# mattreturn1/ComputerVision_ObjectDetection_FeatureMatching

Measured on AMD Instinct MI355X. Metric: matches+homographies/sec (10k x 10k SIFT, 50k RANSAC iters) at 1/2/4/8 GPUs, higher is better.
Workload: dtype i8-MFMA exact-int distances (i32 acc), fp64 DLT/Jacobi, fp32 reprojection; 1 GPU; c4: one global batch of 256 scenes x 1 model set, 10000x10000 descriptors, maxIters 50000, scenes sharded over 1 GPU(s) (256 on rank 0); problems_per_gpu=256, global_batch=256, parallelism=dp1, batches_in_flight=16, dist_backend=nccl, hw_queues=24

## Files before the change

computervision_objectdetection_featurematching_amd/csrc/api.cpp:

```cpp
#include <hip/hip_runtime.h>

#include <algorithm>
#include <cfloat>
#include <climits>
#include <cmath>
#include <cstdarg>
#include <cstdio>
#include <cstdlib>
#include <cstring>
#include <map>
#include <mutex>
#include <string>
#include <vector>

#include "../../include/mim.h"
#include "../../include/mim_detect.hpp"
#include "knn_coll.h"
#include "mim_internal.h"
#include "radius.h"

namespace mim {
void launch_prep_batch(const PrepJob* jobs, int njobs, int total_tiles, hipStream_t st);
void launch_knn(const ProbDev* probs, const KnnWork* works, int n_works, const int* seg_start, int n_blocks, Top2* parts,
                int* dyn_ctr, float kappa, float flip_ratio, hipStream_t st);
// ... 152 lines not shown
        if (err != hipSuccess || ab + bb == 0) return;
        if (ab) memcpy(p + off, a, ab);
        if (bb) memcpy(p + off + ab, b, bb);
        err = hipMemcpyAsync(dst, p + off, ab + bb, hipMemcpyHostToDevice, s);
        off += ab + bb;
    }
    template <class T> void put(const DevBuf& dst, const std::vector<T>& v) { put(dst.p, v.data(), vec_bytes(v)); }
    hipError_t done() { return err != hipSuccess ? err : ps.release_after(s); }
};

}

namespace mim {
struct RansacWs {
    DevBuf state, samples, hyp, counts, bounds, flags, irr_bits, irr, irr_cnt, cls, cls_tab, pass_bits, defer, defer_n, chains, best_h, cand, ncand, cex, cH, decided, stream,
        scratch, inl, tiles, tbox, perm, surv, nsurv, err;
    long long stream_len = 0;
};
}

struct mim_ctx {
    int device = 0;
    hipStream_t own = nullptr, stream = nullptr;
    std::mutex mu;
    std::string err;
    Arena arena;
    std::vector<SetRec> sets;
    DevBuf probs, works, parts, good_q, good_t, pts, n_good, results, masks, knn_idx, knn_dist, inl_tab, inl_out, knn_ctr, ham_works, flt_works;
    RansacWs rws;
    std::vector<ProbDev> h_probs;
    int n_ham_works = 0;
// ... 141 lines not shown
    (void)hipStreamSynchronize(c->stream);
    for (auto& e : c->evs) (void)hipEventDestroy(e.e);
    for (hipEvent_t e : c->ev_pool) (void)hipEventDestroy(e);
    if (c->samp) (void)hipStreamSynchronize(c->samp);
    if (c->ev_samp_fork) (void)hipEventDestroy(c->ev_samp_fork);
    for (auto e : c->ev_samp)
        if (e) (void)hipEventDestroy(e);
    if (c->samp) (void)hipStreamDestroy(c->samp);
    mim::sift_ws_destroy(c->sift);
    for (mim::SiftWs* w : c->sift_scales) mim::sift_ws_destroy(w);
    c->stage.destroy();
    c->prep_stage.destroy();
    c->arena.release();
    for (DevBuf* b : {&c->probs, &c->works, &c->parts, &c->good_q, &c->good_t, &c->pts, &c->n_good,
                      &c->results, &c->masks, &c->knn_idx, &c->knn_dist, &c->inl_tab, &c->inl_out, &c->knn_ctr, &c->ham_works, &c->flt_works, &c->ham_cross_works, &c->colmin, &c->cross_tab, &c->topk_parts, &c->topk_ham_works, &c->topk_flt_works, &c->topk_probs, &c->coll_parts, &c->coll_ham_works, &c->coll_flt_works, &c->coll_i8_probs, &c->coll_i8_works, &c->coll_tab, &c->coll_queries, &c->rad_counts, &c->rad_cursor, &c->rad_offsets, &c->rad_meta, &c->rad_keys, &c->rad_scratch, &c->rad_ham_works, &c->rad_flt_works, &c->rad_i8_works, &c->rad_probs, &c->rws.state, &c->rws.samples,
                      &c->rws.hyp, &c->rws.counts, &c->rws.bounds, &c->rws.flags, &c->rws.irr_bits, &c->rws.irr, &c->rws.irr_cnt, &c->rws.cls, &c->rws.cls_tab, &c->rws.pass_bits, &c->rws.defer, &c->rws.defer_n, &c->rws.chains, &c->rws.best_h, &c->rws.cand, &c->rws.ncand, &c->rws.cex, &c->rws.cH, &c->rws.decided, &c->rws.stream, &c->rws.scratch, &c->rws.inl, &c->rws.tiles, &c->rws.tbox, &c->rws.perm, &c->rws.surv, &c->rws.nsurv, &c->rws.err, &c->prep_jobs})
        b->release();
    if (c->own) (void)hipStreamDestroy(c->own);
    delete c;
}

const char* mim_last_error(const mim_ctx* c) { return c ? c->err.c_str() : "null ctx"; }

mim_status mim_ctx_set_stream(mim_ctx* c, void* stream) {
    if (!c) return MIM_EINVAL;
    std::lock_guard<std::mutex> lk(c->mu);
    c->stream = stream ? (hipStream_t)stream : c->own;
    return MIM_OK;
}

mim_status mim_ctx_set_sampler_stream(mim_ctx* c, int32_t on) {
// ... 1523 lines not shown
    HIPCHK(c, c->rws.defer_n.ensure(sizeof(int) * (size_t)std::max(n, 1) * def_rounds));
    HIPCHK(c, c->rws.chains.ensure(ransac_chain_bytes() * (size_t)std::max(n, 1)));
    HIPCHK(c, c->rws.best_h.ensure(sizeof(double) * 9 * std::max(n, 1)));
    const size_t cap = (size_t)std::max(n, 1) * 2 * kCandPerProblem;
    HIPCHK(c, c->rws.cand.ensure(sizeof(int) * cap));
    HIPCHK(c, c->rws.ncand.ensure(sizeof(int) * 2 * std::max(n, 1)));
    HIPCHK(c, c->rws.cex.ensure(sizeof(int) * cap));
    HIPCHK(c, c->rws.cH.ensure(sizeof(double) * 9 * cap));
    HIPCHK(c, c->rws.decided.ensure(sizeof(int) * cap));
    HIPCHK(c, c->rws.inl.ensure(sizeof(float4) * good_total));
    HIPCHK(c, c->rws.tiles.ensure(sizeof(uint4) * 128 * ((good_total + 31) / 32)));
    HIPCHK(c, c->rws.tbox.ensure(sizeof(float4) * ((good_total + 31) / 32)));
    HIPCHK(c, c->rws.perm.ensure(sizeof(int) * 2 * good_total));
    HIPCHK(c, c->rws.surv.ensure(sizeof(int) * it_total));
    HIPCHK(c, c->rws.nsurv.ensure(sizeof(int) * std::max(n, 1)));
    HIPCHK(c, c->rws.err.ensure(sizeof(int) * 4));
    HIPCHK(c, c->results.ensure(sizeof(mim_result) * std::max(n, 1)));
    HIPCHK(c, c->masks.ensure(good_total));
    HIPCHK(c, hipMemsetAsync(c->rws.err.p, 0, sizeof(int) * 4, c->stream));
    b = RansacBufs{};
    b.state = c->rws.state.as<RansacState>();
    b.samples = c->rws.samples.as<int4>();
    b.hyp = c->rws.hyp.as<float>();
    b.counts = c->rws.counts.as<int>();
    b.bounds = c->rws.bounds.as<int2>();
    b.flags = c->rws.flags.as<uint8_t>();
    b.irr_bits = c->rws.irr_bits.as<uint8_t>();
    b.best_h = c->rws.best_h.as<double>();
    b.cand = c->rws.cand.as<int>();
    b.ncand = c->rws.ncand.as<int>();
// ... 9 lines not shown
    const char* cde = getenv("MIM_CHECK_DEFER");
    b.def_rounds = (cde && cde[0] == '0') ? 0 : def_rounds;
    b.irr_blocks = irr_blocks;
    b.cls = c->rws.cls.as<SamplerClass>();
    b.cls_tab = c->rws.cls_tab.as<SamplerClassSlot>();
    b.cls_tab_n = q_max + 1;
    b.chains = c->rws.chains.p;
    b.stream = c->rws.stream.as<uint32_t>();
    b.stream_len = c->rws.stream_len;
    b.inl = c->rws.inl.as<float4>();
    b.tiles = c->rws.tiles.as<uint4>();
    b.tbox = c->rws.tbox.as<float4>();
    b.perm = c->rws.perm.as<int>();
    b.surv = c->rws.surv.as<int>();
    b.nsurv = c->rws.nsurv.as<int>();
    b.err = c->rws.err.as<int>();
    if (c->samp_on < 0) {
        const char* e = getenv("MIM_SAMPLER_STREAM");
        c->samp_on = (e && e[0] == '0') ? 0 : 1;
    }
    if (c->samp_on && !c->samp) {
        HIPCHK(c, hipStreamCreateWithFlags(&c->samp, hipStreamNonBlocking));
        HIPCHK(c, hipEventCreateWithFlags(&c->ev_samp_fork, hipEventDisableTiming));
        for (auto& e : c->ev_samp) HIPCHK(c, hipEventCreateWithFlags(&e, hipEventDisableTiming));
    }
    b.s2 = c->samp_on ? c->samp : nullptr;
    b.ev_fork = c->ev_samp_fork;
    b.ev_samp[0] = c->ev_samp[0];
    b.ev_samp[1] = c->ev_samp[1];
    rp = RansacParams{};
// ... 19 lines not shown
    g.flag_cap = (long long)np * flag_per;
    g.irr += (long long)p0 * b.irr_blocks * kIrrCap;
    g.irr_cnt += (long long)p0 * b.irr_blocks;
    g.cls += p0;
    g.pass_bits += (long long)p0 * flag_per / 32;
    g.defer += (long long)p0 * b.def_rounds * kRansacDefSlots;
    g.defer_n += (long long)p0 * b.def_rounds;
    g.chains = static_cast<char*>(b.chains) + (size_t)p0 * ransac_chain_bytes();
    g.best_h += 9LL * p0;
    g.cand += (long long)p0 * 2 * kCandPerProblem;
    g.ncand += 2 * p0;
    g.cex += (long long)p0 * 2 * kCandPerProblem;
    g.cH += 9LL * p0 * 2 * kCandPerProblem;
    g.decided += (long long)p0 * 2 * kCandPerProblem;
    g.nsurv += p0;
    ransac_enqueue(rp, np, c->probs.as<ProbDev>() + p0, c->pts.as<float4>(), c->n_good.as<int>() + p0, g,
                   c->masks.as<uint8_t>(), c->results.as<mim_result>() + p0, raw, c->cur, mark_cb, c, c->exact_all);
    HIPCHK(c, hipGetLastError());
    return MIM_OK;
}

static mim_status ransac_locked(mim_ctx* c, int n, const mim_params* prm, int raw) {
    RansacBufs b;
    RansacParams rp;
    long long flag_per = 0;
    mim_status s = ransac_prepare(c, n, prm, b, rp, flag_per);
    if (s != MIM_OK) return s;
    c->cur = c->stream;
    return ransac_enqueue_range(c, 0, n, b, rp, flag_per, raw);
}
// ... 243 lines not shown
```

computervision_objectdetection_featurematching_amd/csrc/mim_internal.h:

```cpp
#pragma once
#include <hip/hip_runtime.h>
#include <stdint.h>

#include "knn_schedule.h"
#include "knn_topk_merge.h"

namespace mim {

constexpr int kDim = 128;
constexpr int kTileRows = 64;
constexpr int kTileBytes = kTileRows * kDim;
constexpr int kNormWords = 4 * kTileRows;
constexpr int kWave = 64;
#ifndef MIM_KNN_STAGE
#define MIM_KNN_STAGE 4
#endif
constexpr int kKnnStage = MIM_KNN_STAGE;

struct SetDev {
    const int8_t* frag;
    const int* norm;
    const float* f32;
    const float2* kp;
    int n;
// ... 179 lines not shown
    int2* defer;
    int* defer_n;
    int def_rounds;
    int irr_blocks;
    SamplerClass* cls;
    SamplerClassSlot* cls_tab;
    int cls_tab_n;
    const uint32_t* stream;
    long long stream_len;
    float4* inl;
    uint4* tiles;
    float4* tbox;
    int* perm;
    int* surv;
    int* nsurv;
    int* err;
    hipStream_t s2;
    hipEvent_t ev_fork;
    hipEvent_t ev_samp[2];
};
}

#include <string>
#include <vector>
#include "../../include/mim.h"
namespace mim {
struct SiftWs;
SiftWs* sift_ws_create();
void sift_ws_destroy(SiftWs* w);
int sift_detect_compute(SiftWs* w, hipStream_t st, const uint8_t* img, int rows, int cols, long long step,
// ... 22 lines not shown
```

computervision_objectdetection_featurematching_amd/csrc/ransac.hip:

```cpp
#include <float.h>

#include <algorithm>
#include <climits>
#include <cstdio>
#include <cstdlib>
#include <vector>

#include "../../include/mim.h"
#include "mim_debug.h"
#include "mim_internal.h"

namespace mim {

__device__ __forceinline__ double d_hypot(double a, double b) {
    a = fabs(a);
    b = fabs(b);
    const bool ab = a > b;
    const double big = ab ? a : b, sm = ab ? b : a;
    const double r = sm / big;
    const double res = big * sqrt(1 + r * r);
    return (ab || b > 0) ? res : 0.0;
}

template <int n> __device__ __forceinline__ int pk(int i, int j) {
// ... 582 lines not shown
    o[0] = c012; o[1] = c21; o[2] = c20; o[3] = c10;
    return fminf(fminf(fabsf(c10), fabsf(c20)), fabsf(c21)) > thr && fabsf(c012) > thr0;
}

__device__ __forceinline__ bool check_subset_fp32(const float* s, const float* d, bool& clear_out) {
    float os[4], od[4];
    const bool cs = set_orient_fp32(s, os), cd = set_orient_fp32(d, od);
    clear_out = cs && cd;
    const unsigned x0 = __float_as_uint(os[0]) ^ __float_as_uint(od[0]);
    const unsigned x1 = __float_as_uint(os[1]) ^ __float_as_uint(od[1]);
    const unsigned x2 = __float_as_uint(os[2]) ^ __float_as_uint(od[2]);
    const unsigned x3 = __float_as_uint(os[3]) ^ __float_as_uint(od[3]);
    return (int)((x0 ^ x1) | (x0 ^ x2) | (x0 ^ x3)) >= 0;
}

__device__ int update_num_iters(double p, double ep, int model_points, int max_iters) {
    p = p > 0. ? p : 0.;
    p = p < 1. ? p : 1.;
    ep = ep > 0. ? ep : 0.;
    ep = ep < 1. ? ep : 1.;
    double num = 1. - p;
    if (num < DBL_MIN) num = DBL_MIN;
    double denom = 1. - pow(1. - ep, (double)model_points);
    if (denom < DBL_MIN) return 0;
    num = log(num);
    denom = log(denom);
    if (denom >= 0 || -num >= max_iters * (-denom)) return max_iters;
    return (int)rint(num / denom);
}

__device__ __forceinline__ unsigned fastmod(unsigned a, unsigned long long M, unsigned d) {
    const unsigned q = __umulhi(a, (unsigned)(M >> 32));
    const unsigned r = a - q * d;
    return min(r, r - d);
}


__device__ __forceinline__ int resolve_at(long long q, const uint32_t* __restrict__ stream, long long slen,
                                          unsigned N, unsigned long long M, int (&idx)[4]) {
    unsigned buf[8];
    long long bq = q, r = q;
#pragma unroll
    for (int k = 0; k < 8; ++k) buf[k] = stream[min(q + k, slen - 1)];
// ... 1747 lines not shown
        }
#pragma unroll
        for (int off = 16; off >= 1; off >>= 1) {
            bx0 = fminf(bx0, __shfl_xor(bx0, off)); bx1 = fmaxf(bx1, __shfl_xor(bx1, off));
            by0 = fminf(by0, __shfl_xor(by0, off)); by1 = fmaxf(by1, __shfl_xor(by1, off));
        }
        if (t < nt && (tid & 31) == 0) {
            const float cx = 0.5f * (bx0 + bx1), cy = 0.5f * (by0 + by1);
            const float rx = fmaxf(bx1 - cx, cx - bx0) * (1.f + 0x1p-22f);
            const float ry = fmaxf(by1 - cy, cy - by0) * (1.f + 0x1p-22f);
            TB[t] = make_float4(cx, cy, rx, ry);
        }
    }
}

enum { kBoundUp = 0, kBoundLoUp = 1, kBoundCap = 2 };

template <int kMode, bool kList>
__global__ __launch_bounds__(kBoundThreads) void ransac_bound_mfma_kernel(const RansacState* __restrict__ st,
                                                                const ProbDev* __restrict__ probs,
                                                                const float4* __restrict__ pts,
                                                                const int4* __restrict__ samples,
                                                                const uint32_t* __restrict__ stream,
                                                                const uint4* __restrict__ tiles,
                                                                int2* __restrict__ bounds, int c0, int c1, int bpp,
                                                                float thr2, int n_probs,
                                                                const float4* __restrict__ tbox,
                                                                int* __restrict__ surv, int* __restrict__ nsurv,
                                                                int list_all) {
    constexpr bool kLo = kMode == kBoundLoUp;
    constexpr bool kCap = kMode == kBoundCap;
    static_assert(!(kList && kMode != kBoundUp), "the survivor list takes the full upper form");
    __shared__ uint4 lt[2][kTileChunk * 128];
    const int xcd = blockIdx.x & 7, j = blockIdx.x >> 3;
    const int p = xcd + 8 * (j / bpp), kb = j % bpp;
    if (p >= n_probs) return;
    const int tid = threadIdx.x, lane = tid & 63;
    const RansacState S = st[p];
    if (!S.active || S.done) return;
    if (kCap && !list_all && S.n < kCapMinN) {
        if (kb == 0 && tid == 0) nsurv[p] = -1;
        return;
    }
    const int n_list0 = kList ? nsurv[p] : 0;
    const bool contig = kList && n_list0 < 0;
    const int n_list = contig ? max(0, min(c1, S.produced) - c0) : n_list0;
    for (int lk = kb * kBoundThreads; !kList || lk < n_list; lk += bpp * kBoundThreads) {
    int it = c0 + kb * kBoundThreads + tid;
    bool act;
    if (kList) {
        act = lk + tid < n_list;
        it = !act ? c0 : contig ? c0 + lk + tid : surv[probs[p].it_off + lk + tid];
    } else {
        if (c0 + kb * kBoundThreads >= min(c1, S.produced)) return;
// ... 61 lines not shown
    const bool lowh = lane < 32;
    const uint4 ux = __builtin_bit_cast(uint4, fx), uy = __builtin_bit_cast(uint4, fy);
    const uint4 uw = __builtin_bit_cast(uint4, fw), un = __builtin_bit_cast(uint4, fn);
    const uint4 s1 = lowh ? un : ux;
    uint4 r1, r2, r3;
    r1.x = __shfl_xor(s1.x, 32); r1.y = __shfl_xor(s1.y, 32); r1.z = __shfl_xor(s1.z, 32); r1.w = __shfl_xor(s1.w, 32);
    r2.x = __shfl_xor(uy.x, 32); r2.y = __shfl_xor(uy.y, 32); r2.z = __shfl_xor(uy.z, 32); r2.w = __shfl_xor(uy.w, 32);
    r3.x = __shfl_xor(uw.x, 32); r3.y = __shfl_xor(uw.y, 32); r3.z = __shfl_xor(uw.z, 32); r3.w = __shfl_xor(uw.w, 32);
    const uint4 zero4 = make_uint4(0, 0, 0, 0);
    const h8v b0x = __builtin_bit_cast(h8v, lowh ? ux : r1);
    const h8v b0y = __builtin_bit_cast(h8v, lowh ? uy : r1);
    const h8v b0w = __builtin_bit_cast(h8v, lowh ? uw : zero4);
    const h8v b1x = __builtin_bit_cast(h8v, lowh ? r1 : un);
    const h8v b1y = __builtin_bit_cast(h8v, lowh ? r2 : un);
    const h8v b1w = __builtin_bit_cast(h8v, lowh ? r3 : zero4);
    const float EK = fmaf(kCap ? (E + C * 0x1p-19f) * (1.f + 1e-6f) : E, (float)kOutScale, 1.f);
    const float ELK = -EL * (float)kOutScale;
    const float Cp = __shfl_xor(C, 32), Ep = __shfl_xor(EK, 32);
    float wa0 = 0.f, wb0 = 0.f, wc0 = 0.f, wa1 = 0.f, wb1 = 0.f, wc1 = 0.f;
    if (kCap) {
        const float wa = count ? (float)h[6] * (float)kOutScale : 0.f;
        const float wb = count ? (float)h[7] * (float)kOutScale : 0.f;
        const float wc = count ? (float)h[8] * (float)kOutScale : 0.f;
        const float wap = __shfl_xor(wa, 32), wbp = __shfl_xor(wb, 32), wcp = __shfl_xor(wc, 32);
        wa0 = lowh ? wa : wap; wb0 = lowh ? wb : wbp; wc0 = lowh ? wc : wcp;
        wa1 = lowh ? wap : wa; wb1 = lowh ? wbp : wb; wc1 = lowh ? wcp : wc;
    }
    const float C0 = lowh ? C : Cp, E0 = lowh ? EK : Ep, C1 = lowh ? Cp : C, E1 = lowh ? Ep : EK;
    float CL0 = 0.f, EL0 = 0.f, CL1 = 0.f, EL1 = 0.f;
    if (kLo) {
        const float CLp = __shfl_xor(CL, 32), ELp = __shfl_xor(ELK, 32);
        CL0 = lowh ? CL : CLp; EL0 = lowh ? ELK : ELp; CL1 = lowh ? CLp : CL; EL1 = lowh ? ELp : ELK;
    }
    const bool wave_counts = __any(count);
    const uint4* __restrict__ T = tiles + (go >> 5) * 128;
// ... 5 lines not shown
        const int tc = min(kTileChunk, nt - t0);
        for (int i0 = wv * 64; i0 < tc * 128; i0 += kBoundThreads)
            __builtin_amdgcn_global_load_lds((const void*)(T + (long long)t0 * 128 + i0 + lane),
                                             (__attribute__((address_space(3))) void*)(lt[buf] + i0), 16, 0, 0);
    };
#ifndef MIM_PROBE_BOUND
#define MIM_PROBE_BOUND 0
#endif
    if (nt > 0) stage(0, 0);
    asm volatile("s_waitcnt vmcnt(0)" ::: "memory");
    __syncthreads();
    for (int t0 = 0, buf = 0; t0 < (MIM_PROBE_BOUND == 2 ? 0 : nt); t0 += kTileChunk, buf ^= 1) {
        const int tc = min(kTileChunk, nt - t0);
        if (t0 + kTileChunk < nt) stage(t0 + kTileChunk, buf ^ 1);
        if (wave_counts && MIM_PROBE_BOUND == 0) {
          if (kCap) {
            float4 bx[kTileChunk];
#pragma unroll
            for (int t = 0; t < kTileChunk; ++t) bx[t] = TB[min(t0 + t, nt - 1)];
#pragma unroll
            for (int t = 0; t < kTileChunk; ++t)
                asm volatile("" : "+s"(bx[t].x), "+s"(bx[t].y), "+s"(bx[t].z), "+s"(bx[t].w));
#pragma unroll
            for (int t = 0; t < kTileChunk; ++t) {
                if (t >= tc) break;
                const h8v ax = __builtin_bit_cast(h8v, lt[buf][t * 128 + lane]);
                const h8v ay = __builtin_bit_cast(h8v, lt[buf][t * 128 + 64 + lane]);
                const f16acc zc = {};
                const f16acc ex0 = __builtin_amdgcn_mfma_f32_32x32x16_f16(ax, b0x, zc, 0, 0, 0);
                const f16acc ey0 = __builtin_amdgcn_mfma_f32_32x32x16_f16(ay, b0y, zc, 0, 0, 0);
                const f16acc ex1 = __builtin_amdgcn_mfma_f32_32x32x16_f16(ax, b1x, zc, 0, 0, 0);
                const f16acc ey1 = __builtin_amdgcn_mfma_f32_32x32x16_f16(ay, b1y, zc, 0, 0, 0);
                const float R0 = fmaf(C0, fmaf(fabsf(wa0), bx[t].z, fmaf(fabsf(wb0), bx[t].w,
                                          fabsf(fmaf(wa0, bx[t].x, fmaf(wb0, bx[t].y, wc0))))), E0);
                const float R1 = fmaf(C1, fmaf(fabsf(wa1), bx[t].z, fmaf(fabsf(wb1), bx[t].w,
                                          fabsf(fmaf(wa1, bx[t].x, fmaf(wb1, bx[t].y, wc1))))), E1);
#pragma unroll
                for (int r = 0; r < 16; ++r) {
                    keep0 += clamp01((R0 - fabsf(ex0[r])) - fabsf(ey0[r]));
                    keep1 += clamp01((R1 - fabsf(ex1[r])) - fabsf(ey1[r]));
                }
            }
          } else
          for (int t = 0; t < tc; ++t) {
            const h8v ax = __builtin_bit_cast(h8v, lt[buf][t * 128 + lane]);
            const h8v ay = __builtin_bit_cast(h8v, lt[buf][t * 128 + 64 + lane]);
            const f16acc zc = {};
            const f16acc ex0 = __builtin_amdgcn_mfma_f32_32x32x16_f16(ax, b0x, zc, 0, 0, 0);
            const f16acc ey0 = __builtin_amdgcn_mfma_f32_32x32x16_f16(ay, b0y, zc, 0, 0, 0);
            const f16acc w0 = __builtin_amdgcn_mfma_f32_32x32x16_f16(ax, b0w, zc, 0, 0, 0);
            const f16acc ex1 = __builtin_amdgcn_mfma_f32_32x32x16_f16(ax, b1x, zc, 0, 0, 0);
            const f16acc ey1 = __builtin_amdgcn_mfma_f32_32x32x16_f16(ay, b1y, zc, 0, 0, 0);
            const f16acc w1 = __builtin_amdgcn_mfma_f32_32x32x16_f16(ax, b1w, zc, 0, 0, 0);
#pragma unroll
            for (int r = 0; r < 16; ++r) {
// ... 111 lines not shown
    }
}

constexpr int kCandWaves = 16;
constexpr int kCandCap = kCandWaves * 64;
static_assert(kCandCap == kCandPerProblem, "candidate list layout shared with api.cpp");

constexpr int kCandThreads = 1024;

__device__ __forceinline__ int wave_isum(int v) {
#pragma unroll
    for (int off = 32; off >= 1; off >>= 1) v += __shfl_xor(v, off);
    return v;
}

constexpr int kPreWaves = 16;

__global__ __launch_bounds__(64) void ransac_prescreen_kernel(const RansacState* __restrict__ st,
                                                              const ProbDev* __restrict__ probs,
                                                              const int2* __restrict__ bounds,
                                                              const float4* __restrict__ pts,
                                                              const int4* __restrict__ samples,
                                                              const uint32_t* __restrict__ stream,
                                                              const int* __restrict__ cand,
                                                              const int* __restrict__ ncand, int* __restrict__ cex,
                                                              double* __restrict__ cH, int* __restrict__ decided,
                                                              float thr2, int L, int cap) {
    const int p = blockIdx.x / kPreWaves, j = blockIdx.x % kPreWaves, lane = threadIdx.x;
    const RansacState S = st[p];
    if (!S.active || S.done) return;
    const ProbDev PD = probs[p];
    const int2* Bd = bounds + PD.it_off;
    const long long lb = (long long)(2 * p + L) * kCandCap;
    const int nl = min(ncand[2 * p + L], cap);
    const float4* __restrict__ P = pts + PD.good_off;
    const int n = S.n;
    for (int k = j; k < nl; k += kPreWaves) {
        const int t = cand[lb + k];
        const int2 bd = Bd[t];
        int res = 0, cnt = 0;
        if (bd.x == bd.y) {
            res = 1;
            cnt = bd.x;
        } else {
            const int4 s4 = decode_sample(samples[PD.it_off + t], stream, (unsigned)n, S.modM);
            double Hd[8];
            bool invalid = false, uncertain = false;
            float eta = 0.f;
            double eta_model = 0;
            bound_hypothesis(P, s4, Hd, invalid, uncertain, eta, eta_model);
            if (!invalid && !uncertain) {
                float tt = thr2 + fmaf(1e-7f * S.smax, S.smax, 0.5f);
                float tl = thr2 - fmaf(1e-7f * S.smax, S.smax, 0.5f);
                if (eta > 0.f) {
                    const float wd = S.smax * fmaf(eta * eta, S.smax, 10.2f * eta);
                    tt += wd;
                    tl -= wd;
                }
                const double mx = ldexp(1.0, -ilogb((double)S.sa)), mu = ldexp(1.0, -ilogb((double)S.sb));
                const double gam = 4.0 * 0x1p-24 + fmin(eta_model, 1.0);
                const double ax = fmax((fabs(Hd[0]) + fabs(Hd[1])) * mx + fabs(Hd[2]),
                                       (fabs(Hd[3]) + fabs(Hd[4])) * mx + fabs(Hd[5]));
                const double aw = (fabs(Hd[6]) + fabs(Hd[7])) * mx + 1.0;
                const double A = gam * (ax + (mu + 6.0) * aw) * (1.0 + 1e-6);
                const double TT = (double)tt * (1.0 + 1e-9), TL = (double)fmaxf(tl, 0.f) * (1.0 - 1e-9);
                int in = 0, unc = 0;
                for (int i = lane; i < n; i += 64) {
                    const float4 q = P[i];
                    const double x = q.x, y = q.y;
                    const double W = fma(Hd[6], x, fma(Hd[7], y, 1.0));
                    const double X = fma(Hd[0], x, fma(Hd[1], y, Hd[2]));
                    const double Y = fma(Hd[3], x, fma(Hd[4], y, Hd[5]));
                    const double ex = fabs(X - (double)q.z * W), ey = fabs(Y - (double)q.w * W);
                    const double ux = fmax(ex - A, 0.0), uy = fmax(ey - A, 0.0);
                    const double W2 = W * W;
                    const bool maybe = ux * ux + uy * uy <= TT * W2;
                    const bool surely = (ex + A) * (ex + A) + (ey + A) * (ey + A) < TL * W2;
                    in += surely ? 1 : 0;
                    unc += (maybe && !surely) ? 1 : 0;
                }
                in = wave_isum(in);
                unc = wave_isum(unc);
                if (unc == 0) {
                    res = 1;
                    cnt = in;
                }
            }
        }
        if (lane == 0) {
            decided[lb + k] = res;
            if (res) {
                cex[lb + k] = cnt;
// ... 97 lines not shown
                               sd + threadIdx.x, thr2, H);
    atomicAdd(stats + 0, 1ull);
    if (ex != cex[lb + k]) {
        atomicAdd(stats + 1, 1ull);
        const int2 bd = bounds[probs[p].it_off + t];
        printf("[mim] prescreen mismatch p=%d it=%d exact=%d prescreen=%d lo=%d hi=%d n=%d\n", p, t, ex, cex[lb + k],
               bd.x, bd.y, S.n);
    }
}


__global__ __launch_bounds__(kCandThreads) void ransac_cand_kernel(RansacState* __restrict__ st,
                                                                   const ProbDev* __restrict__ probs,
                                                                   const int2* __restrict__ bounds, int c1,
                                                                   int* __restrict__ cand, int* __restrict__ ncand,
                                                                   int L, int cap) {
    __shared__ int wred[kCandThreads / 64], wred2[kCandThreads / 64];
    const int p = blockIdx.x, tid = threadIdx.x;
    const RansacState S = st[p];
    if (!S.active || S.done) {
        if (tid == 0) ncand[2 * p + L] = 0;
        return;
    }
    const int2* Bd = bounds + probs[p].it_off;
    const int t0 = S.next_iter, t1 = max(t0, min(min(c1, S.produced), S.niters));
    const int ch = (t1 - t0 + kCandThreads - 1) / kCandThreads;
    const int a = min(t1, t0 + tid * ch), e = min(t1, a + ch);
    constexpr int kB = 16;
    int lmax = INT_MIN;
    for (int t = a; t < e; t += kB) {
        int2 v[kB];
#pragma unroll
        for (int k = 0; k < kB; ++k) v[k] = Bd[min(t + k, e - 1)];
#pragma unroll
        for (int k = 0; k < kB; ++k) {
            lmax = t + k < e ? max(lmax, v[k].x) : lmax;
        }
    }
    const int init = max(3, max(S.max_good, S.lo_max));
    int all;
    const int run0 = block_excl_max(lmax, init, wred, all);
    int cnt = 0, run = run0;
    for (int t = a; t < e; t += kB) {
        int2 v[kB];
#pragma unroll
        for (int k = 0; k < kB; ++k) v[k] = Bd[min(t + k, e - 1)];
#pragma unroll
        for (int k = 0; k < kB; ++k) {
            if (t + k < e) {
                cnt += v[k].y > run;
                run = max(run, v[k].x);
            }
        }
    }
    int total;
    int o = block_excl_sum(cnt, wred2, total);
    if (cnt && o < cap) {
        int* C = cand + (long long)(2 * p + L) * kCandCap;
        run = run0;
        for (int t = a; t < e && o < cap; ++t) {
            const int2 b = Bd[t];
            if (b.y > run) C[o++] = t;
            run = max(run, b.x);
        }
    }
    if (tid == 0) {
        ncand[2 * p + L] = total;
        st[p].lo_max = max(S.lo_max, all);
        if (L == 0) st[p].defer = 0;
    }
}

constexpr int kExactGroups = 4;
constexpr int kExactWaves = kCandCap / kExactGroups;

#ifndef MIM_EXACT_OCC
#define MIM_EXACT_OCC 1
#endif
__global__ __launch_bounds__(64, MIM_EXACT_OCC) void ransac_exact_kernel(const RansacState* __restrict__ st,
                                                          const ProbDev* __restrict__ probs,
                                                          const float4* __restrict__ pts,
                                                          const int4* __restrict__ samples,
                                                          const uint32_t* __restrict__ stream,
                                                          const int* __restrict__ cand, const int* __restrict__ ncand,
// ... 761 lines not shown
    if (n_probs <= 0) return;
    ransac_init_kernel<<<(n_probs + 255) / 256, 256, 0, s>>>(b.state, n_good, n_probs, prm.max_iters, prm.min_good,
                                                             b.best_h);
    const int max_iters = prm.max_iters > 1 ? prm.max_iters : 1;
    const char* sw = getenv("MIM_SAMPLER_WALK");
    const int use_chain = !(sw && sw[0] == '1');
    int first = max_iters <= 4096 ? 512 : 4096;
    if (const char* fc = getenv("MIM_FIRST_CHUNK")) first = std::max(1, atoi(fc));
    int c0 = 0, chunk = first;
    const float thr2 = (float)(prm.thresh * prm.thresh);
    if (!exact_all) ransac_tiles_kernel<<<n_probs, 256, 0, s>>>(b.state, probs, pts, b.tiles, b.tbox, b.perm, b.nsurv);
    const char* bce = getenv("MIM_BOUND_CAP");
    const int bound_cap = (bce && bce[0] == '0') ? 0 : 1;
    const char* bae = getenv("MIM_BOUND_CAP_ALL");
    const int cap_all = (bae && bae[0] == '1') ? 1 : 0;
    const bool split = b.s2 && !exact_all;
    hipStream_t ss = split ? b.s2 : s;
    if (split) {
        (void)hipEventRecord(b.ev_fork, s);
        (void)hipStreamWaitEvent(ss, b.ev_fork, 0);
        mark(mark_ctx, "fork", ss);
    }
    int ci = 0, c1_first = 0;
    const int cap = prm.cand_cap > 0 ? std::min(prm.cand_cap, kCandCap) : kCandCap;
    const char* pe = getenv("MIM_PRESCREEN");
    const int prescreen = (pe && pe[0] == '0') ? 0 : 1;
    const char* se = getenv("MIM_SETTLE");
    const int settle = (se && se[0] == '0') ? 0 : 1;
    const char* we = getenv("MIM_WINNER_H");
    const int winner_h = !we ? 2 : we[0] == '1' ? 1 : we[0] == '0' ? 0 : 2;
// ... 78 lines not shown
            ransac_select_kernel<<<n_probs, 64, 0, s>>>(b.state, probs, b.counts, c1, prm.conf);
            mark(mark_ctx, "select", s);
            if (getenv("MIM_DEBUG_TRACE") && n_probs == 1) {
                std::vector<int> hc(c1 - c0);
                std::vector<int4> hs(c1 - c0);
                (void)hipMemcpyAsync(hc.data(), b.counts + c0, sizeof(int) * (c1 - c0), hipMemcpyDeviceToHost, s);
                (void)hipMemcpyAsync(hs.data(), b.samples + c0, sizeof(int4) * (c1 - c0), hipMemcpyDeviceToHost, s);
                (void)hipStreamSynchronize(s);
                for (int i = 0; i < c1 - c0; ++i)
                    fprintf(stderr, "[trace] %d %d %d %d %d %d\n", c0 + i, hc[i], hs[i].x, hs[i].y, hs[i].z, hs[i].w);
            }
        } else {
            if (c0 == 0)
                ransac_bound_mfma_kernel<kBoundLoUp, false><<<8 * ((n_probs + 7) / 8) * bppb, kBoundThreads, 0, s>>>(
                    b.state, probs, pts, b.samples, b.stream, b.tiles, b.bounds, c0, c1, bppb, thr2, n_probs, b.tbox,
                    b.surv, b.nsurv, 0);
            else if (!bound_cap)
                ransac_bound_mfma_kernel<kBoundUp, false><<<8 * ((n_probs + 7) / 8) * bppb, kBoundThreads, 0, s>>>(
                    b.state, probs, pts, b.samples, b.stream, b.tiles, b.bounds, c0, c1, bppb, thr2, n_probs, b.tbox,
                    b.surv, b.nsurv, 0);
            else {
                const int bppl = std::min(bppb, kSurvBlocks);
                ransac_bound_mfma_kernel<kBoundCap, false><<<8 * ((n_probs + 7) / 8) * bppb, kBoundThreads, 0, s>>>(
                    b.state, probs, pts, b.samples, b.stream, b.tiles, b.bounds, c0, c1, bppb, thr2, n_probs, b.tbox,
                    b.surv, b.nsurv, cap_all);
                ransac_bound_mfma_kernel<kBoundUp, true><<<8 * ((n_probs + 7) / 8) * bppl, kBoundThreads, 0, s>>>(
                    b.state, probs, pts, b.samples, b.stream, b.tiles, b.bounds, c0, c1, bppl, thr2, n_probs, b.tbox,
                    b.surv, b.nsurv, 0);
                if (getenv("MIM_DEBUG_NSURV")) {
                    std::vector<int> h(n_probs);
                    (void)hipMemcpyAsync(h.data(), b.nsurv, sizeof(int) * n_probs, hipMemcpyDeviceToHost, s);
                    (void)hipStreamSynchronize(s);
                    long long sum = 0; int mx = 0, small = 0;
                    for (int i = 0; i < n_probs; ++i) {
                        sum += std::max(h[i], 0);
                        mx = std::max(mx, h[i]);
                        small += h[i] < 0;
                    }
                    fprintf(stderr, "[mim] chunk [%d,%d): survivors mean %.1f max %d (%d small problems on the full bound alone)\n",
                            c0, c1, (double)sum / n_probs, mx, small);
                }
            }
            mark(mark_ctx, "score", s);
// ... 2 lines not shown
                unsigned long long h[6] = {0, 0, 0, 0, 0, 0};
                if (hipMalloc(&dst, sizeof h) == hipSuccess) {
                    (void)hipMemsetAsync(dst, 0, sizeof h, s);
                    const int bpp64 = (c1 - c0 + 63) / 64;
                    ransac_bound_check_kernel<<<n_probs * bpp64, 64, 0, s>>>(b.state, probs, pts, b.samples, b.stream,
                                                                             b.bounds, c0, c1, bpp64, thr2, dst);
                    (void)hipMemcpyAsync(h, dst, sizeof h, hipMemcpyDeviceToHost, s);
                    (void)hipStreamSynchronize(s);
                    (void)hipFree(dst);
                }
                fprintf(stderr, "[mim] bound check chunk [%d,%d): checked %llu lo_viol %llu hi_viol %llu valid_mismatch %llu "
                        "mean_width %.2f tight %llu\n", c0, c1, h[0], h[1], h[2], h[3], h[0] ? (double)h[4] / h[0] : 0.0, h[5]);
            }
            const int L = c0 == 0 ? 0 : 1;
            ransac_cand_kernel<<<n_probs, kCandThreads, 0, s>>>(b.state, probs, b.bounds, c1, b.cand, b.ncand, L,
                                                                cap);
            if (prescreen) {
                ransac_prescreen_kernel<<<n_probs * kPreWaves, 64, 0, s>>>(b.state, probs, b.bounds, pts, b.samples,
                                                                          b.stream, b.cand, b.ncand, b.cex, b.cH,
                                                                          b.decided, thr2, L, cap);
                if (settle)
                    ransac_settle_kernel<<<n_probs, 64, 0, s>>>(b.state, probs, b.bounds, b.cand, b.ncand, b.cex, b.cH,
                                                                b.decided, L, cap, winner_h);
            }
            mark(mark_ctx, "cand", s);
            if (prescreen && getenv("MIM_CHECK_PRESCREEN")) {
                unsigned long long* dst = nullptr;
                unsigned long long h[2] = {0, 0};
                if (hipMalloc(&dst, sizeof h) == hipSuccess) {
                    (void)hipMemsetAsync(dst, 0, sizeof h, s);
                    ransac_prescreen_check_kernel<<<n_probs * (kCandCap / 64), 64, 0, s>>>(
// ... 39 lines not shown
        std::vector<RansacState> hs(n_probs);
        (void)hipMemcpyAsync(bh.data(), b.best_h, sizeof(double) * bh.size(), hipMemcpyDeviceToHost, s);
        (void)hipMemcpyAsync(hs.data(), b.state, sizeof(RansacState) * n_probs, hipMemcpyDeviceToHost, s);
        (void)hipStreamSynchronize(s);
        int with = 0, without = 0;
        for (int i = 0; i < n_probs; ++i)
            if (hs[i].active && hs[i].best_iter >= 0 && hs[i].n >= kSmallMaxN) (bh[9 * i + 8] != 0.0 ? with : without)++;
        fprintf(stderr, "[mim] best_h: %d problems with the exact pass's fp64 bestModel, %d without\n", with, without);
    }
    ransac_refine_kernel<<<(n_probs + kRW - 1) / kRW, kRT, 0, s>>>(b.state, probs, pts, n_good, b.samples, b.stream, b.inl,
                                                                  masks, results, prm, raw, b.best_h, exact_all, n_probs);
    mark(mark_ctx, "refine", s);
}

}
```

Measured before the change: 38760 problems/s.

## Add strip-bound prefilter and pilot bar to prune RANSAC bound stage

Adds a cheap single-axis (x-residual only) MFMA bound pass, then a pilot kernel that exactly counts sure inliers for the best strip survivor. It raises the candidate bar to the level below which the iteration count cannot drop, and lists survivors above that bar. When the list is small the full capped bound pass is skipped for that problem, and the raised bar feeds the candidate kernel. This aims to cut MFMA work and candidate counts in later chunks, at the cost of two extra kernel launches and possible fallback work when the strip list overflows.

```diff
diff --git a/computervision_objectdetection_featurematching_amd/csrc/api.cpp b/computervision_objectdetection_featurematching_amd/csrc/api.cpp
--- a/computervision_objectdetection_featurematching_amd/csrc/api.cpp
+++ b/computervision_objectdetection_featurematching_amd/csrc/api.cpp
@@ -190,7 +190,7 @@
 namespace mim {
 struct RansacWs {
     DevBuf state, samples, hyp, counts, bounds, flags, irr_bits, irr, irr_cnt, cls, cls_tab, pass_bits, defer, defer_n, chains, best_h, cand, ncand, cex, cH, decided, stream,
-        scratch, inl, tiles, tbox, perm, surv, nsurv, err;
+        scratch, inl, tiles, tbox, perm, surv, nsurv, strip, err;
     long long stream_len = 0;
 };
 }
@@ -362,7 +362,7 @@
     c->arena.release();
     for (DevBuf* b : {&c->probs, &c->works, &c->parts, &c->good_q, &c->good_t, &c->pts, &c->n_good,
                       &c->results, &c->masks, &c->knn_idx, &c->knn_dist, &c->inl_tab, &c->inl_out, &c->knn_ctr, &c->ham_works, &c->flt_works, &c->ham_cross_works, &c->colmin, &c->cross_tab, &c->topk_parts, &c->topk_ham_works, &c->topk_flt_works, &c->topk_probs, &c->coll_parts, &c->coll_ham_works, &c->coll_flt_works, &c->coll_i8_probs, &c->coll_i8_works, &c->coll_tab, &c->coll_queries, &c->rad_counts, &c->rad_cursor, &c->rad_offsets, &c->rad_meta, &c->rad_keys, &c->rad_scratch, &c->rad_ham_works, &c->rad_flt_works, &c->rad_i8_works, &c->rad_probs, &c->rws.state, &c->rws.samples,
-                      &c->rws.hyp, &c->rws.counts, &c->rws.bounds, &c->rws.flags, &c->rws.irr_bits, &c->rws.irr, &c->rws.irr_cnt, &c->rws.cls, &c->rws.cls_tab, &c->rws.pass_bits, &c->rws.defer, &c->rws.defer_n, &c->rws.chains, &c->rws.best_h, &c->rws.cand, &c->rws.ncand, &c->rws.cex, &c->rws.cH, &c->rws.decided, &c->rws.stream, &c->rws.scratch, &c->rws.inl, &c->rws.tiles, &c->rws.tbox, &c->rws.perm, &c->rws.surv, &c->rws.nsurv, &c->rws.err, &c->prep_jobs})
+                      &c->rws.hyp, &c->rws.counts, &c->rws.bounds, &c->rws.flags, &c->rws.irr_bits, &c->rws.irr, &c->rws.irr_cnt, &c->rws.cls, &c->rws.cls_tab, &c->rws.pass_bits, &c->rws.defer, &c->rws.defer_n, &c->rws.chains, &c->rws.best_h, &c->rws.cand, &c->rws.ncand, &c->rws.cex, &c->rws.cH, &c->rws.decided, &c->rws.stream, &c->rws.scratch, &c->rws.inl, &c->rws.tiles, &c->rws.tbox, &c->rws.perm, &c->rws.surv, &c->rws.nsurv, &c->rws.strip, &c->rws.err, &c->prep_jobs})
         b->release();
     if (c->own) (void)hipStreamDestroy(c->own);
     delete c;
@@ -1916,6 +1916,7 @@
     HIPCHK(c, c->rws.perm.ensure(sizeof(int) * 2 * good_total));
     HIPCHK(c, c->rws.surv.ensure(sizeof(int) * it_total));
     HIPCHK(c, c->rws.nsurv.ensure(sizeof(int) * std::max(n, 1)));
+    HIPCHK(c, c->rws.strip.ensure(sizeof(int4) * std::max(n, 1)));
     HIPCHK(c, c->rws.err.ensure(sizeof(int) * 4));
     HIPCHK(c, c->results.ensure(sizeof(mim_result) * std::max(n, 1)));
     HIPCHK(c, c->masks.ensure(good_total));
@@ -1955,6 +1956,7 @@
     b.perm = c->rws.perm.as<int>();
     b.surv = c->rws.surv.as<int>();
     b.nsurv = c->rws.nsurv.as<int>();
+    b.strip = c->rws.strip.as<int4>();
     b.err = c->rws.err.as<int>();
     if (c->samp_on < 0) {
         const char* e = getenv("MIM_SAMPLER_STREAM");
@@ -2004,6 +2006,7 @@
     g.cH += 9LL * p0 * 2 * kCandPerProblem;
     g.decided += (long long)p0 * 2 * kCandPerProblem;
     g.nsurv += p0;
+    g.strip += p0;
     ransac_enqueue(rp, np, c->probs.as<ProbDev>() + p0, c->pts.as<float4>(), c->n_good.as<int>() + p0, g,
                    c->masks.as<uint8_t>(), c->results.as<mim_result>() + p0, raw, c->cur, mark_cb, c, c->exact_all);
     HIPCHK(c, hipGetLastError());
diff --git a/computervision_objectdetection_featurematching_amd/csrc/mim_internal.h b/computervision_objectdetection_featurematching_amd/csrc/mim_internal.h
--- a/computervision_objectdetection_featurematching_amd/csrc/mim_internal.h
+++ b/computervision_objectdetection_featurematching_amd/csrc/mim_internal.h
@@ -217,6 +217,7 @@
     int* perm;
     int* surv;
     int* nsurv;
+    int4* strip;
     int* err;
     hipStream_t s2;
     hipEvent_t ev_fork;
diff --git a/computervision_objectdetection_featurematching_amd/csrc/ransac.hip b/computervision_objectdetection_featurematching_amd/csrc/ransac.hip
--- a/computervision_objectdetection_featurematching_amd/csrc/ransac.hip
+++ b/computervision_objectdetection_featurematching_amd/csrc/ransac.hip
@@ -620,7 +620,7 @@
     return (int)((x0 ^ x1) | (x0 ^ x2) | (x0 ^ x3)) >= 0;
 }
 
-__device__ int update_num_iters(double p, double ep, int model_points, int max_iters) {
+__host__ __device__ int update_num_iters(double p, double ep, int model_points, int max_iters) {
     p = p > 0. ? p : 0.;
     p = p < 1. ? p : 1.;
     ep = ep > 0. ? ep : 0.;
@@ -633,6 +633,15 @@
     denom = log(denom);
     if (denom >= 0 || -num >= max_iters * (-denom)) return max_iters;
     return (int)rint(num / denom);
+}
+
+__host__ __device__ inline int free_level(int n, double conf, int max_iters) {
+    int lo = 0, hi = n + 1;
+    while (hi - lo > 1) {
+        const int c = lo + (hi - lo) / 2;
+        if (update_num_iters(conf, (double)(n - c) / n, 4, max_iters) == max_iters) lo = c; else hi = c;
+    }
+    return lo;
 }
 
 __device__ __forceinline__ unsigned fastmod(unsigned a, unsigned long long M, unsigned d) {
@@ -2410,7 +2419,7 @@
     }
 }
 
-enum { kBoundUp = 0, kBoundLoUp = 1, kBoundCap = 2 };
+enum { kBoundUp = 0, kBoundLoUp = 1, kBoundCap = 2, kBoundStrip = 3, kBoundCapRest = 4 };
 
 template <int kMode, bool kList>
 __global__ __launch_bounds__(kBoundThreads) void ransac_bound_mfma_kernel(const RansacState* __restrict__ st,
@@ -2423,9 +2432,11 @@
                                                                 float thr2, int n_probs,
                                                                 const float4* __restrict__ tbox,
                                                                 int* __restrict__ surv, int* __restrict__ nsurv,
-                                                                int list_all) {
+                                                                int list_all, const int4* __restrict__ strip) {
     constexpr bool kLo = kMode == kBoundLoUp;
-    constexpr bool kCap = kMode == kBoundCap;
+    constexpr bool kCap = kMode == kBoundCap || kMode == kBoundCapRest;
+    constexpr bool kStrip = kMode == kBoundStrip;
+    constexpr bool kCapR = kCap || kStrip;
     static_assert(!(kList && kMode != kBoundUp), "the survivor list takes the full upper form");
     __shared__ uint4 lt[2][kTileChunk * 128];
     const int xcd = blockIdx.x & 7, j = blockIdx.x >> 3;
@@ -2434,6 +2445,8 @@
     const int tid = threadIdx.x, lane = tid & 63;
     const RansacState S = st[p];
     if (!S.active || S.done) return;
+    if (kStrip && S.n < kCapMinN) return;
+    if (kMode == kBoundCapRest && strip[p].y) return;
     if (kCap && !list_all && S.n < kCapMinN) {
         if (kb == 0 && tid == 0) nsurv[p] = -1;
         return;
@@ -2525,11 +2538,11 @@
     const h8v b1x = __builtin_bit_cast(h8v, lowh ? r1 : un);
     const h8v b1y = __builtin_bit_cast(h8v, lowh ? r2 : un);
     const h8v b1w = __builtin_bit_cast(h8v, lowh ? r3 : zero4);
-    const float EK = fmaf(kCap ? (E + C * 0x1p-19f) * (1.f + 1e-6f) : E, (float)kOutScale, 1.f);
+    const float EK = fmaf(kCapR ? (E + C * 0x1p-19f) * (1.f + 1e-6f) : E, (float)kOutScale, 1.f);
     const float ELK = -EL * (float)kOutScale;
     const float Cp = __shfl_xor(C, 32), Ep = __shfl_xor(EK, 32);
     float wa0 = 0.f, wb0 = 0.f, wc0 = 0.f, wa1 = 0.f, wb1 = 0.f, wc1 = 0.f;
-    if (kCap) {
+    if (kCapR) {
         const float wa = count ? (float)h[6] * (float)kOutScale : 0.f;
         const float wb = count ? (float)h[7] * (float)kOutScale : 0.f;
         const float wc = count ? (float)h[8] * (float)kOutScale : 0.f;
@@ -2565,7 +2578,7 @@
         const int tc = min(kTileChunk, nt - t0);
         if (t0 + kTileChunk < nt) stage(t0 + kTileChunk, buf ^ 1);
         if (wave_counts && MIM_PROBE_BOUND == 0) {
-          if (kCap) {
+          if (kCapR) {
             float4 bx[kTileChunk];
 #pragma unroll
             for (int t = 0; t < kTileChunk; ++t) bx[t] = TB[min(t0 + t, nt - 1)];
@@ -2574,22 +2587,23 @@
                 asm volatile("" : "+s"(bx[t].x), "+s"(bx[t].y), "+s"(bx[t].z), "+s"(bx[t].w));
 #pragma unroll
             for (int t = 0; t < kTileChunk; ++t) {
+                if (kStrip && t >= tc) continue;
                 if (t >= tc) break;
                 const h8v ax = __builtin_bit_cast(h8v, lt[buf][t * 128 + lane]);
                 const h8v ay = __builtin_bit_cast(h8v, lt[buf][t * 128 + 64 + lane]);
                 const f16acc zc = {};
                 const f16acc ex0 = __builtin_amdgcn_mfma_f32_32x32x16_f16(ax, b0x, zc, 0, 0, 0);
-                const f16acc ey0 = __builtin_amdgcn_mfma_f32_32x32x16_f16(ay, b0y, zc, 0, 0, 0);
+                const f16acc ey0 = kStrip ? zc : __builtin_amdgcn_mfma_f32_32x32x16_f16(ay, b0y, zc, 0, 0, 0);
                 const f16acc ex1 = __builtin_amdgcn_mfma_f32_32x32x16_f16(ax, b1x, zc, 0, 0, 0);
-                const f16acc ey1 = __builtin_amdgcn_mfma_f32_32x32x16_f16(ay, b1y, zc, 0, 0, 0);
+                const f16acc ey1 = kStrip ? zc : __builtin_amdgcn_mfma_f32_32x32x16_f16(ay, b1y, zc, 0, 0, 0);
                 const float R0 = fmaf(C0, fmaf(fabsf(wa0), bx[t].z, fmaf(fabsf(wb0), bx[t].w,
                                           fabsf(fmaf(wa0, bx[t].x, fmaf(wb0, bx[t].y, wc0))))), E0);
                 const float R1 = fmaf(C1, fmaf(fabsf(wa1), bx[t].z, fmaf(fabsf(wb1), bx[t].w,
                                           fabsf(fmaf(wa1, bx[t].x, fmaf(wb1, bx[t].y, wc1))))), E1);
 #pragma unroll
                 for (int r = 0; r < 16; ++r) {
-                    keep0 += clamp01((R0 - fabsf(ex0[r])) - fabsf(ey0[r]));
-                    keep1 += clamp01((R1 - fabsf(ex1[r])) - fabsf(ey1[r]));
+                    keep0 += clamp01(kStrip ? R0 - fabsf(ex0[r]) : (R0 - fabsf(ex0[r])) - fabsf(ey0[r]));
+                    keep1 += clamp01(kStrip ? R1 - fabsf(ex1[r]) : (R1 - fabsf(ex1[r])) - fabsf(ey1[r]));
                 }
             }
           } else
@@ -2731,6 +2745,44 @@
     return v;
 }
 
+struct DiscTest {
+    double Hd[8], A, TT, TL;
+    __device__ bool setup(const float4* __restrict__ P, int4 s4, const RansacState& S, float thr2) {
+        bool invalid = false, uncertain = false;
+        float eta = 0.f;
+        double eta_model = 0;
+        bound_hypothesis(P, s4, Hd, invalid, uncertain, eta, eta_model);
+        if (invalid || uncertain) return false;
+        float tt = thr2 + fmaf(1e-7f * S.smax, S.smax, 0.5f);
+        float tl = thr2 - fmaf(1e-7f * S.smax, S.smax, 0.5f);
+        if (eta > 0.f) {
+            const float wd = S.smax * fmaf(eta * eta, S.smax, 10.2f * eta);
+            tt += wd;
+            tl -= wd;
+        }
+        const double mx = ldexp(1.0, -ilogb((double)S.sa)), mu = ldexp(1.0, -ilogb((double)S.sb));
+        const double gam = 4.0 * 0x1p-24 + fmin(eta_model, 1.0);
+        const double ax = fmax((fabs(Hd[0]) + fabs(Hd[1])) * mx + fabs(Hd[2]),
+                               (fabs(Hd[3]) + fabs(Hd[4])) * mx + fabs(Hd[5]));
+        const double aw = (fabs(Hd[6]) + fabs(Hd[7])) * mx + 1.0;
+        A = gam * (ax + (mu + 6.0) * aw) * (1.0 + 1e-6);
+        TT = (double)tt * (1.0 + 1e-9);
+        TL = (double)fmaxf(tl, 0.f) * (1.0 - 1e-9);
+        return true;
+    }
+    __device__ __forceinline__ void point(const float4 q, bool& surely, bool& maybe) const {
+        const double x = q.x, y = q.y;
+        const double W = fma(Hd[6], x, fma(Hd[7], y, 1.0));
+        const double X = fma(Hd[0], x, fma(Hd[1], y, Hd[2]));
+        const double Y = fma(Hd[3], x, fma(Hd[4], y, Hd[5]));
+        const double ex = fabs(X - (double)q.z * W), ey = fabs(Y - (double)q.w * W);
+        const double ux = fmax(ex - A, 0.0), uy = fmax(ey - A, 0.0);
+        const double W2 = W * W;
+        maybe = ux * ux + uy * uy <= TT * W2;
+        surely = (ex + A) * (ex + A) + (ey + A) * (ey + A) < TL * W2;
+    }
+};
+
 constexpr int kPreWaves = 16;
 
 __global__ __launch_bounds__(64) void ransac_prescreen_kernel(const RansacState* __restrict__ st,
@@ -2761,38 +2813,12 @@
             cnt = bd.x;
         } else {
             const int4 s4 = decode_sample(samples[PD.it_off + t], stream, (unsigned)n, S.modM);
-            double Hd[8];
-            bool invalid = false, uncertain = false;
-            float eta = 0.f;
-            double eta_model = 0;
-            bound_hypothesis(P, s4, Hd, invalid, uncertain, eta, eta_model);
-            if (!invalid && !uncertain) {
-                float tt = thr2 + fmaf(1e-7f * S.smax, S.smax, 0.5f);
-                float tl = thr2 - fmaf(1e-7f * S.smax, S.smax, 0.5f);
-                if (eta > 0.f) {
-                    const float wd = S.smax * fmaf(eta * eta, S.smax, 10.2f * eta);
-                    tt += wd;
-                    tl -= wd;
-                }
-                const double mx = ldexp(1.0, -ilogb((double)S.sa)), mu = ldexp(1.0, -ilogb((double)S.sb));
-                const double gam = 4.0 * 0x1p-24 + fmin(eta_model, 1.0);
-                const double ax = fmax((fabs(Hd[0]) + fabs(Hd[1])) * mx + fabs(Hd[2]),
-                                       (fabs(Hd[3]) + fabs(Hd[4])) * mx + fabs(Hd[5]));
-                const double aw = (fabs(Hd[6]) + fabs(Hd[7])) * mx + 1.0;
-                const double A = gam * (ax + (mu + 6.0) * aw) * (1.0 + 1e-6);
-                const double TT = (double)tt * (1.0 + 1e-9), TL = (double)fmaxf(tl, 0.f) * (1.0 - 1e-9);
+            DiscTest D;
+            if (D.setup(P, s4, S, thr2)) {
                 int in = 0, unc = 0;
                 for (int i = lane; i < n; i += 64) {
-                    const float4 q = P[i];
-                    const double x = q.x, y = q.y;
-                    const double W = fma(Hd[6], x, fma(Hd[7], y, 1.0));
-                    const double X = fma(Hd[0], x, fma(Hd[1], y, Hd[2]));
-                    const double Y = fma(Hd[3], x, fma(Hd[4], y, Hd[5]));
-                    const double ex = fabs(X - (double)q.z * W), ey = fabs(Y - (double)q.w * W);
-                    const double ux = fmax(ex - A, 0.0), uy = fmax(ey - A, 0.0);
-                    const double W2 = W * W;
-                    const bool maybe = ux * ux + uy * uy <= TT * W2;
-                    const bool surely = (ex + A) * (ex + A) + (ey + A) * (ey + A) < TL * W2;
+                    bool surely, maybe;
+                    D.point(P[i], surely, maybe);
                     in += surely ? 1 : 0;
                     unc += (maybe && !surely) ? 1 : 0;
                 }
@@ -2920,7 +2946,7 @@
                                                                    const ProbDev* __restrict__ probs,
                                                                    const int2* __restrict__ bounds, int c1,
                                                                    int* __restrict__ cand, int* __restrict__ ncand,
-                                                                   int L, int cap) {
+                                                                   int L, int cap, const int4* __restrict__ strip) {
     __shared__ int wred[kCandThreads / 64], wred2[kCandThreads / 64];
     const int p = blockIdx.x, tid = threadIdx.x;
     const RansacState S = st[p];
@@ -2945,7 +2971,7 @@
     }
     const int init = max(3, max(S.max_good, S.lo_max));
     int all;
-    const int run0 = block_excl_max(lmax, init, wred, all);
+    const int run0 = max(block_excl_max(lmax, init, wred, all), strip ? strip[p].x : 0);
     int cnt = 0, run = run0;
     for (int t = a; t < e; t += kB) {
         int2 v[kB];
@@ -2974,6 +3000,104 @@
         ncand[2 * p + L] = total;
         st[p].lo_max = max(S.lo_max, all);
         if (L == 0) st[p].defer = 0;
+    }
+}
+
+constexpr int kPilotThreads = 1024;
+constexpr int kPilots = kPilotThreads / 64;
+constexpr int kStripListDiv = 16;
+
+__device__ int surely_in_count(const float4* __restrict__ P, int n, int4 s4, const RansacState& S, float thr2) {
+    DiscTest D;
+    if (!D.setup(P, s4, S, thr2)) return -1;
+    int in = 0;
+    for (int i = (threadIdx.x & 63); i < n; i += 64) {
+        bool surely, maybe;
+        D.point(P[i], surely, maybe);
+        in += surely ? 1 : 0;
+    }
+    return wave_isum(in);
+}
+
+__global__ __launch_bounds__(kPilotThreads) void ransac_strip_pilot_kernel(const RansacState* __restrict__ st,
+                                                                           const ProbDev* __restrict__ probs,
+                                                                           const int2* __restrict__ bounds,
+                                                                           const float4* __restrict__ pts,
+                                                                           const int4* __restrict__ samples,
+                                                                           const uint32_t* __restrict__ stream,
+                                                                           int c0, int c1, float thr2, double conf,
+                                                                           int max_iters, int* __restrict__ surv,
+                                                                           int* __restrict__ nsurv,
+                                                                           int4* __restrict__ strip) {
+    __shared__ int wtop[kPilots];
+    __shared__ int s_bar, s_B, s_top, s_cnt;
+    const int p = blockIdx.x, tid = threadIdx.x, lane = tid & 63, wv = tid >> 6;
+    const RansacState S = st[p];
+    if (!S.active || S.done || S.n < kCapMinN) {
+        if (tid == 0) strip[p] = make_int4(0, 0, 0, 0);
+        return;
+    }
+    const ProbDev PD = probs[p];
+    const int2* __restrict__ Bd = bounds + PD.it_off;
+    const int n = S.n;
+    const int t1 = min(min(c1, S.produced), S.niters);
+    unsigned long long key = 0;
+    for (int t = c0 + tid; t < t1; t += kPilotThreads) {
+        const int2 b = Bd[t];
+        if (b.x == 0 && b.y > 0 && b.y < n) {
+            const unsigned long long k = ((unsigned long long)(unsigned)b.y << 32) | (unsigned)~t;
+            key = k > key ? k : key;
+        }
+    }
+#pragma unroll
+    for (int off = 32; off >= 1; off >>= 1) {
+        const unsigned hi = __shfl_xor((unsigned)(key >> 32), off), lo = __shfl_xor((unsigned)key, off);
+        const unsigned long long k = ((unsigned long long)hi << 32) | lo;
+        key = k > key ? k : key;
+    }
+    int low = 0;
+    if (key) {
+        const int t = (int)~(unsigned)key;
+        low = surely_in_count(pts + PD.good_off, n, decode_sample(samples[PD.it_off + t], stream, (unsigned)n, S.modM),
+                              S, thr2);
+    }
+    if (lane == 0) wtop[wv] = low;
+    __syncthreads();
+    if (tid == 0) {
+        int top = 0;
+        for (int w = 0; w < kPilots; ++w) top = max(top, wtop[w]);
+        int B = 0;
+        if (top > 1 && S.niters == max(max_iters, 1)) B = max(0, min(top, free_level(n, conf, S.niters)) - 1);
+        const int bar0 = max(3, max(S.max_good, S.lo_max));
+        s_B = B > bar0 ? B : 0;
+        s_top = top;
+        s_bar = max(bar0, B);
+        s_cnt = 0;
+    }
+    __syncthreads();
+    const int bar = s_bar, limit = (t1 - c0) / kStripListDiv;
+    int* __restrict__ SV = surv + PD.it_off;
+    for (int tb = c0; tb < t1; tb += kPilotThreads) {
+        const int t = tb + tid;
+        bool on = false;
+        if (t < t1) {
+            const int2 b = Bd[t];
+            on = b.x == 0 && b.y > bar;
+        }
+        const unsigned long long m = __ballot(on);
+        if (m) {
+            int base = 0;
+            if (lane == 0) base = atomicAdd(&s_cnt, __popcll(m));
+            base = __shfl(base, 0);
+            const int pos = base + __popcll(m & ((1ull << lane) - 1));
+            if (on && pos < limit) SV[pos] = t;
+        }
+    }
+    __syncthreads();
+    if (tid == 0) {
+        const int cnt = s_cnt, stand = cnt <= limit ? 1 : 0;
+        nsurv[p] = stand ? cnt : 0;
+        strip[p] = make_int4(stand ? s_B : 0, stand, cnt, s_top);
     }
 }
 
@@ -3765,6 +3889,8 @@
     const int bound_cap = (bce && bce[0] == '0') ? 0 : 1;
     const char* bae = getenv("MIM_BOUND_CAP_ALL");
     const int cap_all = (bae && bae[0] == '1') ? 1 : 0;
+    const char* bse = getenv("MIM_BOUND_STRIP");
+    const int strip = bound_cap && !cap_all && max_iters > 4096 && !(bse && bse[0] == '0');
     const bool split = b.s2 && !exact_all;
     hipStream_t ss = split ? b.s2 : s;
     if (split) {
@@ -3873,19 +3999,48 @@
             if (c0 == 0)
                 ransac_bound_mfma_kernel<kBoundLoUp, false><<<8 * ((n_probs + 7) / 8) * bppb, kBoundThreads, 0, s>>>(
                     b.state, probs, pts, b.samples, b.stream, b.tiles, b.bounds, c0, c1, bppb, thr2, n_probs, b.tbox,
-                    b.surv, b.nsurv, 0);
+                    b.surv, b.nsurv, 0, nullptr);
             else if (!bound_cap)
                 ransac_bound_mfma_kernel<kBoundUp, false><<<8 * ((n_probs + 7) / 8) * bppb, kBoundThreads, 0, s>>>(
                     b.state, probs, pts, b.samples, b.stream, b.tiles, b.bounds, c0, c1, bppb, thr2, n_probs, b.tbox,
-                    b.surv, b.nsurv, 0);
+                    b.surv, b.nsurv, 0, nullptr);
             else {
                 const int bppl = std::min(bppb, kSurvBlocks);
+                if (strip) {
+                    ransac_bound_mfma_kernel<kBoundStrip, false><<<8 * ((n_probs + 7) / 8) * bppb, kBoundThreads, 0, s>>>(
+                        b.state, probs, pts, b.samples, b.stream, b.tiles, b.bounds, c0, c1, bppb, thr2, n_probs,
+                        b.tbox, b.surv, b.nsurv, 0, nullptr);
+                    ransac_strip_pilot_kernel<<<n_probs, kPilotThreads, 0, s>>>(b.state, probs, b.bounds, pts, b.samples,
+                                                                               b.stream, c0, c1, thr2, prm.conf,
+                                                                               prm.max_iters, b.surv, b.nsurv, b.strip);
+                    ransac_bound_mfma_kernel<kBoundCapRest, false><<<8 * ((n_probs + 7) / 8) * bppb, kBoundThreads, 0, s>>>(
+                        b.state, probs, pts, b.samples, b.stream, b.tiles, b.bounds, c0, c1, bppb, thr2, n_probs,
+                        b.tbox, b.surv, b.nsurv, 0, b.strip);
+                    if (getenv("MIM_DEBUG_NSURV")) {
+                        std::vector<int4> h(n_probs);
+                        (void)hipMemcpyAsync(h.data(), b.strip, sizeof(int4) * n_probs, hipMemcpyDeviceToHost, s);
+                        (void)hipStreamSynchronize(s);
+                        int stand = 0, raised = 0; long long sum = 0, bsum = 0;
+                        for (int i = 0; i < n_probs; ++i) {
+                            stand += h[i].y;
+                            raised += h[i].x > 0;
+                            sum += h[i].y ? h[i].z : 0;
+                            bsum += h[i].x;
+                        }
+                        fprintf(stderr, "[mim] chunk [%d,%d): strip stands for %d of %d problems (listed mean %.1f), "
+                                "capped stage for %d; pilot bar on %d (mean %.1f)\n", c0, c1, stand, n_probs,
+                                stand ? (double)sum / stand : 0.0, n_probs - stand, raised, raised ? (double)bsum / raised : 0.0);
+                        if (n_probs == 1)
+                            fprintf(stderr, "[mim] chunk [%d,%d): problem 0: %d iterations above the bar, largest pilot count %d\n",
+                                    c0, c1, h[0].z, h[0].w);
+                    }
+                } else
                 ransac_bound_mfma_kernel<kBoundCap, false><<<8 * ((n_probs + 7) / 8) * bppb, kBoundThreads, 0, s>>>(
                     b.state, probs, pts, b.samples, b.stream, b.tiles, b.bounds, c0, c1, bppb, thr2, n_probs, b.tbox,
-                    b.surv, b.nsurv, cap_all);
+                    b.surv, b.nsurv, cap_all, nullptr);
                 ransac_bound_mfma_kernel<kBoundUp, true><<<8 * ((n_probs + 7) / 8) * bppl, kBoundThreads, 0, s>>>(
                     b.state, probs, pts, b.samples, b.stream, b.tiles, b.bounds, c0, c1, bppl, thr2, n_probs, b.tbox,
-                    b.surv, b.nsurv, 0);
+                    b.surv, b.nsurv, 0, nullptr);
                 if (getenv("MIM_DEBUG_NSURV")) {
                     std::vector<int> h(n_probs);
                     (void)hipMemcpyAsync(h.data(), b.nsurv, sizeof(int) * n_probs, hipMemcpyDeviceToHost, s);
@@ -3918,7 +4073,7 @@
             }
             const int L = c0 == 0 ? 0 : 1;
             ransac_cand_kernel<<<n_probs, kCandThreads, 0, s>>>(b.state, probs, b.bounds, c1, b.cand, b.ncand, L,
-                                                                cap);
+                                                                cap, c0 > 0 && strip ? b.strip : nullptr);
             if (prescreen) {
                 ransac_prescreen_kernel<<<n_probs * kPreWaves, 64, 0, s>>>(b.state, probs, b.bounds, pts, b.samples,
                                                                           b.stream, b.cand, b.ncand, b.cex, b.cH,
@@ -3988,3 +4143,8 @@
 }
 
 }
+
+extern "C" int32_t mim_test_ransac_free_level(int32_t n, double confidence, int32_t max_iters) {
+    if (n < 1 || max_iters < 1) return 0;
+    return mim::free_level(n, confidence, max_iters);
+}
```

Result: faster. 43040 problems/s, median of 6 (+11.0%).
